# kouyt5/lightning-asr

Hardware: AMD Instinct MI355X
Metric: audio-seconds/sec training (asr13x1, bs=32, 10 s clips) (higher is better)
Workload: dtype bf16; 1 GPU; asr13x1 QuartzNet-CTC train step, bs=32/GPU, 10 s synthetic 16 kHz clips, labels.txt vocab (C=28), HIP mel+conv+CTC+NovoGrad, random-init weights; global_batch=32, n_class=28, parallelism=dp1, feature_prefetch=True, hip_graph=True, staged_backward=False

## Files before the change

### lightning_asr_amd/csrc/conv.hip

```cpp
#include "common.h"
#include "fused.h"

namespace lasr {

static thread_local const DwTapCtx* g_dw_tap_ctx = nullptr;
void dw_taps_set_ctx(const DwTapCtx* ctx) { g_dw_tap_ctx = ctx; }
bool dw_taps_enabled() {
  static const bool on = !(getenv("LASR_DW_TAPS") && atoi(getenv("LASR_DW_TAPS")) == 0);
  return on;
}
const uint32_t* dw_taps_for(const float* w, int flip, int64_t C) {
  (void)flip;
  const DwTapCtx* c = g_dw_tap_ctx;
  if (!c || C % 64 != 0) return nullptr;
  for (int i = 0; i < c->n; ++i)
    if (c->w[i] == w && c->C[i] == (int)C) return c->t[i];
  return nullptr;
}

static constexpr int kCB = 64;
static constexpr int kTT = 128;
static constexpr int kR = 8;
static constexpr int kMaxK = 128;

// ... 718 lines not shown
  __builtin_amdgcn_s_waitcnt(0);
#endif
  DW_STAMP(3);
}

template <int NKS, int NSET>
__global__ __launch_bounds__(512, 1) void dwconv_s1_mfma_kernel(const bf16_t* __restrict__ x, const float* __restrict__ w,
                                                                const bf16_t* __restrict__ addend, bf16_t* __restrict__ y,
                                                                int Tlen, int C, int k, int flip, const uint32_t* __restrict__ taps) {
  extern __shared__ __attribute__((aligned(16))) char smem_raw[];
  dwconv_s1_mfma_body<NKS, NSET>(x, w, addend, y, Tlen, C, k, flip, blockIdx.x, blockIdx.y, blockIdx.z, gridDim.z, smem_raw, taps);
}

template <int NKS, int NSET>
__global__ __launch_bounds__(512, 1) void dwconv_s1_mfma_bn_kernel(DwBnIn bn, const float* __restrict__ w, bf16_t* __restrict__ y, int Tlen,
                                                                   int C, int k, const uint32_t* __restrict__ taps) {
  extern __shared__ __attribute__((aligned(16))) char smem_raw[];
  dwconv_s1_mfma_body<NKS, NSET, true>(nullptr, w, nullptr, y, Tlen, C, k, 0, blockIdx.x, blockIdx.y, blockIdx.z, gridDim.z, smem_raw, taps, bn);
}

static constexpr int kSub = 32;

template <typename T>
__global__ __launch_bounds__(256) void dwconv_wgrad_s1_kernel(const T* __restrict__ x, const T* __restrict__ dy,
                                                              float* __restrict__ partials, int64_t Tlen, int64_t C, int k,
                                                              int ts) {
  extern __shared__ __attribute__((aligned(16))) char smem_raw[];
  const int pad = k / 2;
  const int ng = (k + 7) >> 3;
  const int kpad = ng * 8;
  const int WT = kSub * ts;
  const int in_rows = WT + kpad + 8;
  using P = S1<T>;
  constexpr int LD = P::kTileLd;
  T* s_x = reinterpret_cast<T*>(smem_raw);
  T* s_d = s_x + (size_t)in_rows * LD;
  const int b = blockIdx.z;
  const int64_t c0 = (int64_t)blockIdx.y * kCB;
  const int cl = threadIdx.x & 15, grp = threadIdx.x >> 4;
  const int jg = grp % ng, sp = grp / ng;
  const bool active = sp < ts;
  const T* xb = x + (int64_t)b * Tlen * C;
  const T* db = dy + (int64_t)b * Tlen * C;
  float4 acc[8];
#pragma unroll
  for (int j = 0; j < 8; ++j) acc[j] = make_float4(0.f, 0.f, 0.f, 0.f);
  const int64_t tbeg = (int64_t)blockIdx.x * kWChunk;
  const int64_t tend = tbeg + kWChunk < Tlen ? tbeg + kWChunk : Tlen;
  for (int64_t t0 = tbeg; t0 < tend; t0 += WT) {
    __syncthreads();
    const int64_t in0 = t0 - pad;
    {
      constexpr int kXP = (3 * kSub + kMaxK + 8 + P::kRowsPerPass - 1) / P::kRowsPerPass, kDP = (3 * kSub + P::kRowsPerPass - 1) / P::kRowsPerPass;
      const int lr = threadIdx.x / P::kLanesPerRow, lc = (threadIdx.x % P::kLanesPerRow) * P::kVec;
      const bool c_in = c0 + lc < C;
      uint4 vx[kXP], vd[kDP];
#pragma unroll
      for (int p = 0; p < kXP; ++p) {
        const int r = lr + p * P::kRowsPerPass;
        const int64_t ti = in0 + r;
        const uint4 ld = *reinterpret_cast<const uint4*>(xb + (int64_t)min(max(ti, (int64_t)0), Tlen - 1) * C + min(c0 + lc, C - P::kVec));
        const uint32_t mk = (r < in_rows && c_in && ti >= 0 && ti < Tlen) ? 0xffffffffu : 0u;
        vx[p] = make_uint4(ld.x & mk, ld.y & mk, ld.z & mk, ld.w & mk);
      }
#pragma unroll
      for (int p = 0; p < kDP; ++p) {
        const int r = lr + p * P::kRowsPerPass;
        const int64_t t = t0 + r;
        const uint4 ld = *reinterpret_cast<const uint4*>(db + (int64_t)min(t, Tlen - 1) * C + min(c0 + lc, C - P::kVec));
        const uint32_t mk = (r < WT && c_in && t < tend) ? 0xffffffffu : 0u;
        vd[p] = make_uint4(ld.x & mk, ld.y & mk, ld.z & mk, ld.w & mk);
      }
#pragma unroll
      for (int p = 0; p < kXP; ++p) {
        const int r = lr + p * P::kRowsPerPass;
        if (r < in_rows) *reinterpret_cast<uint4*>(s_x + (size_t)r * LD + lc) = vx[p];
      }
#pragma unroll
      for (int p = 0; p < kDP; ++p) {
        const int r = lr + p * P::kRowsPerPass;
        if (r < WT) *reinterpret_cast<uint4*>(s_d + (size_t)r * LD + lc) = vd[p];
      }
    }
    __syncthreads();
    if (active) {
      const T* xs = s_x + (size_t)(sp * kSub + jg * 8) * LD + cl * 4;
      const T* ds = s_d + (size_t)(sp * kSub) * LD + cl * 4;
      float4 win[8];
#pragma unroll
      for (int i = 0; i < 7; ++i) win[i] = lds_ld4<T>(xs + (size_t)i * LD);
      for (int tq = 0; tq < kSub; tq += 8) {
#pragma unroll
        for (int tt = 0; tt < 8; ++tt) {
          win[(tt + 7) & 7] = lds_ld4<T>(xs + (size_t)(tq + tt + 7) * LD);
          const float4 dv = lds_ld4<T>(ds + (size_t)(tq + tt) * LD);
#pragma unroll
          for (int jj = 0; jj < 8; ++jj) {
            const float4 xv = win[(tt + jj) & 7];
            acc[jj].x = fmaf(dv.x, xv.x, acc[jj].x);
            acc[jj].y = fmaf(dv.y, xv.y, acc[jj].y);
            acc[jj].z = fmaf(dv.z, xv.z, acc[jj].z);
            acc[jj].w = fmaf(dv.w, xv.w, acc[jj].w);
          }
        }
      }
    }
  }
  __syncthreads();
  float* s_red = reinterpret_cast<float*>(smem_raw);
  if (active) {
#pragma unroll
    for (int jj = 0; jj < 8; ++jj)
      *reinterpret_cast<float4*>(s_red + ((size_t)(sp * kpad + jg * 8 + jj)) * kCB + cl * 4) = acc[jj];
  }
  __syncthreads();
  float* out = partials + ((int64_t)b * gridDim.x + blockIdx.x) * C * k;
  for (int i = threadIdx.x; i < k * kCB; i += 256) {
    const int ch = i / k, j = i - ch * k;
    if (c0 + ch < C) {
      float s = 0.f;
      for (int q = 0; q < ts; ++q) s += s_red[((size_t)(q * kpad + j)) * kCB + ch];
      out[(c0 + ch) * k + j] = s;
    }
  }
}

namespace dwg {
static constexpr int TU = 288;
static constexpr int XF = TU + 16 * 7 + 8;
static constexpr int DF = TU + 16;
static constexpr int LDX = XF * 2;
static constexpr int LDD = DF * 2 + 16;
static constexpr int RSG = 256;
static constexpr int X_OFF = 0, D0_OFF = kCB * LDX;
static constexpr int ST_OFF = D0_OFF + kCB * LDD;
static constexpr int SMEM = ST_OFF + RSG * dwm::LDST;
static constexpr int XR = (XF + RSG - 1) / RSG, DR = (DF + RSG - 1) / RSG;
}

__device__ __forceinline__ void dwconv_wgrad_s1_mfma_body(const bf16_t* __restrict__ x, const bf16_t* __restrict__ dy,
                                                          float* __restrict__ partials, int Tlen, int C, int k, int bx, int by,
                                                          int bz, int gz, char* smem_raw) {
  using namespace dwg;
  char* ximg = smem_raw + X_OFF;
  char* d0 = smem_raw + D0_OFF;
  char* stage = smem_raw + ST_OFF;
  const int tid = threadIdx.x, lane = tid & 63, wid = tid >> 6;
  const int b = by, c0 = bx * kCB;
  const int pad = k / 2, P = (pad + 7) & ~7, sh = P - pad;
  const int n16 = lane & 15, g4 = lane >> 4;
  const bf16_t* xb = x + (size_t)b * Tlen * C;
  const bf16_t* db = dy + (size_t)b * Tlen * C;
  typedef __attribute__((address_space(3))) dw_s16x4 lds_s4;

  dw_f32x4 acc[8];
#pragma unroll
  for (int ch = 0; ch < 8; ++ch) acc[ch] = dw_f32x4{0.f, 0.f, 0.f, 0.f};
  for (int i = tid; i < kCB * 4; i += 512) *reinterpret_cast<uint32_t*>(d0 + (i >> 2) * LDD + DF * 2 + (i & 3) * 4) = 0u;

  const int n_tiles = (Tlen + 15 + TU) / TU;
  DW_STAMP(0);
  uint4 v[XR + DR][4];
  auto issue_loads = [&](int q) {
#pragma unroll
    for (int r = 0; r < XR + DR; ++r) {
#pragma unroll
      for (int h = 0; h < 4; ++h) {
        const int chk = tid + 512 * h;
        const bool isx = r < XR;
        const int fr = (isx ? r : r - XR) * RSG + (chk >> 3);
        const int t = isx ? TU * q + fr - P : TU * q - 16 + fr;
        const int cc = c0 + ((chk & 7) << 3);
        const bool ok = fr < (isx ? XF : DF) && t >= 0 && t < Tlen && cc < C;
        const bf16_t* src = isx ? xb : db;
        const uint4 ld = *reinterpret_cast<const uint4*>(src + (size_t)min(max(t, 0), Tlen - 1) * C + min(cc, C - 8));
        const uint32_t mk = ok ? 0xffffffffu : 0u;
        v[r][h] = make_uint4(ld.x & mk, ld.y & mk, ld.z & mk, ld.w & mk);
      }
    }
  };
  const int zq = bz, zn = gz;
  issue_loads(zq);
  for (int q = zq; q < n_tiles; q += zn) {
#pragma unroll
    for (int r = 0; r < XR + DR; ++r) {
      const bool isx = r < XR;
      const int rr = isx ? r : r - XR;
      __syncthreads();
#pragma unroll
      for (int h = 0; h < 4; ++h) {
        const int chk = tid + 512 * h;
        *reinterpret_cast<uint4*>(stage + (chk >> 3) * dwm::LDST + ((chk & 7) << 4)) = v[r][h];
      }
      __syncthreads();
      char* img = isx ? ximg : d0;
      const int ldi = isx ? LDX : LDD, nfr = isx ? XF : DF;
#pragma unroll
      for (int it = 0; it < 8; ++it) {
        const int blk = wid * 8 + it;
        const int fb = (blk >> 2) * 16 + g4 * 4, cg = blk & 3;
        const int qq = n16 >> 2, pp = n16 & 3;
        const dw_s16x4 d = __builtin_amdgcn_ds_read_tr16_b64_v4i16((lds_s4*)(stage + (fb + qq) * dwm::LDST + (cg * 16 + pp * 4) * 2));
        const int fr = rr * RSG + fb;
        if (fr < nfr) *reinterpret_cast<dw_s16x4*>(img + (cg * 16 + n16) * ldi + fr * 2) = d;
      }
    }
    __syncthreads();
    if (q == zq) DW_STAMP(1);
    if (q + zn < n_tiles) issue_loads(q + zn);
    if (q == zq) DW_STAMP(2);

#pragma unroll
    for (int ch = 0; ch < 8; ++ch) {
      const int cl = wid * 8 + ch;
      const int e0 = 8 * g4 - n16 + 16;
      const uint32_t shft = (e0 & 1) * 16;
      const uint32_t* arow = reinterpret_cast<const uint32_t*>(d0 + cl * LDD) + (e0 >> 1);
      const char* brow = ximg + cl * LDX + (16 * n16 + 8 * g4) * 2;
#pragma unroll
      for (int kb = 0; kb < TU / 32; kb += 3) {
        uint32_t wa[3][5];
        uint4 bb[3];
#pragma unroll
        for (int j = 0; j < 3; ++j) {
#pragma unroll
          for (int i = 0; i < 5; ++i) wa[j][i] = arow[16 * (kb + j) + i];
          bb[j] = *reinterpret_cast<const uint4*>(brow + 64 * (kb + j));
        }
#pragma unroll
        for (int j = 0; j < 3; ++j) {
          union { uint32_t u[4]; dw_bf16x8 v; } af, bf;
#pragma unroll
          for (int i = 0; i < 4; ++i) af.u[i] = __builtin_amdgcn_alignbit(wa[j][i + 1], wa[j][i], shft);
          bf.u[0] = bb[j].x; bf.u[1] = bb[j].y; bf.u[2] = bb[j].z; bf.u[3] = bb[j].w;
          acc[ch] = __builtin_amdgcn_mfma_f32_16x16x32_bf16(af.v, bf.v, acc[ch], 0, 0, 0);
        }
      }
    }
  }
  DW_STAMP(3);
  float* out = partials + ((size_t)b * zn + zq) * C * k;
#pragma unroll
  for (int ch = 0; ch < 8; ++ch) {
    const int c = c0 + wid * 8 + ch;
#pragma unroll
    for (int r = 0; r < 4; ++r) {
      const int j = 16 * n16 + 4 * g4 + r - sh;
      if (c < C && j >= 0 && j < k) out[(size_t)c * k + j] = acc[ch][r];
    }
  }
}

__global__ __launch_bounds__(512, 1) void dwconv_wgrad_s1_mfma_kernel(const bf16_t* __restrict__ x, const bf16_t* __restrict__ dy,
                                                                      float* __restrict__ partials, int Tlen, int C, int k) {
  extern __shared__ __attribute__((aligned(16))) char smem_raw[];
  dwconv_wgrad_s1_mfma_body(x, dy, partials, Tlen, C, k, blockIdx.x, blockIdx.y, blockIdx.z, gridDim.z, smem_raw);
}

struct DwBwd {
  const bf16_t* x; const bf16_t* dy; const float* w; const bf16_t* addend; bf16_t* dx; float* partials;
  int Tlen, C, k;
  int gx, B, gz_w, gz_d, n_w;
};
template <int NKS, int NSET>
__global__ __launch_bounds__(512, 1) void dwconv_bwd_s1_mfma_kernel(DwBwd a) {
  extern __shared__ __attribute__((aligned(16))) char smem_raw[];
  int id = blockIdx.x;
  if (id < a.n_w) {
    const int bx = id % a.gx, by = (id / a.gx) % a.B, bz = id / (a.gx * a.B);
    dwconv_wgrad_s1_mfma_body(a.x, a.dy, a.partials, a.Tlen, a.C, a.k, bx, by, bz, a.gz_w, smem_raw);
  } else {
    id -= a.n_w;
    const int bx = id % a.gx, by = (id / a.gx) % a.B, bz = id / (a.gx * a.B);
    dwconv_s1_mfma_body<NKS, NSET>(a.dy, a.w, a.addend, a.dx, a.Tlen, a.C, a.k, 1, bx, by, bz, a.gz_d, smem_raw, nullptr);
  }
}


__device__ __forceinline__ uint32_t dpp_row_shl(uint32_t v, int n) {
  switch (n) {
    case 0: return v;
    case 2: return (uint32_t)__builtin_amdgcn_update_dpp(0, (int)v, 0x102, 0xf, 0xf, true);
    case 4: return (uint32_t)__builtin_amdgcn_update_dpp(0, (int)v, 0x104, 0xf, 0xf, true);
    case 6: return (uint32_t)__builtin_amdgcn_update_dpp(0, (int)v, 0x106, 0xf, 0xf, true);
    case 8: return (uint32_t)__builtin_amdgcn_update_dpp(0, (int)v, 0x108, 0xf, 0xf, true);
    default: __builtin_unreachable();
  }
}

namespace dwu {
static constexpr int TT = 256;
static constexpr int FR = 384;
static constexpr int LDI = 784;
static constexpr int RS = 128;
template <int NKS, int NW>
struct Cfg {
  static constexpr int CB = 8 * NW, NT = 64 * NW;
  static constexpr int LDST = NW == 8 ? 160 : 96;
  static constexpr int WROW = 2 * (16 * NKS + 16);
  static constexpr int D_OFF = 0, X_OFF = CB * LDI, ST_OFF = 2 * CB * LDI, W_OFF = ST_OFF + RS * LDST;
  static constexpr int SMEM = W_OFF + CB * WROW * 4;
  static constexpr int LDO = CB * 2 + 16, LDOF = CB * 4 + 16;
  static_assert(TT * LDOF <= ST_OFF, "output image fits the two input images");
};
}

struct DwUni {
  const bf16_t* x; const bf16_t* dy; const float* w; const bf16_t* addend; bf16_t* dx; float* partials;
  int Tlen, C, k, gx, B, gz, total;
  const uint32_t* taps;
};

template <int NKS, int NW, bool NTL = false>
__global__ __launch_bounds__(64 * NW, NW == 8 ? 1 : 2) void dwconv_bwd_uni_kernel(DwUni a) {
  using K = dwu::Cfg<NKS, NW>;
  using namespace dwu;
  constexpr int CB = K::CB, NT = K::NT, LDST = K::LDST, WROW = K::WROW, HALF = WROW / 2, CG = CB / 16;
  extern __shared__ __attribute__((aligned(16))) char smem_raw[];
  int L;
  {
    const int id = blockIdx.x, xcd = id & 7, slot = id >> 3;
    L = NW == 8 ? id : (((slot >> 1) * 8 + xcd) * 2 + (slot & 1));
  }
  if (L >= a.total) return;
  const int bx = L % a.gx, by = (L / a.gx) % a.B, bz = L / (a.gx * a.B), gz = a.gz;
  char* dimg = smem_raw + K::D_OFF;
  char* ximg = smem_raw + K::X_OFF;
  char* stage = smem_raw + K::ST_OFF;
  uint32_t* wsm = reinterpret_cast<uint32_t*>(smem_raw + K::W_OFF);
  const int tid = threadIdx.x, lane = tid & 63, wid = tid >> 6;
  const int Tlen = a.Tlen, C = a.C, k = a.k;
  const int b = by, c0 = bx * CB;
  const int pad = k / 2, P = (pad + 7) & ~7, sh = P - pad;
  const int n16 = lane & 15, g4 = lane >> 4;
  const bf16_t* xb = a.x + (size_t)b * Tlen * C;
  const bf16_t* db = a.dy + (size_t)b * Tlen * C;
  const bf16_t* addend = a.addend;
  typedef __attribute__((address_space(3))) dw_s16x4 lds_s4;

  dw_f32x4 accw[8];
#pragma unroll
  for (int ch = 0; ch < 8; ++ch) accw[ch] = dw_f32x4{0.f, 0.f, 0.f, 0.f};

  const int n_tiles = (Tlen + TT - 1) / TT;
  constexpr int kRounds = FR / RS;
  uint4 vd[kRounds][2], vx[kRounds][2], ra[4];
  auto issue_loads = [&](int q) {
    const int tA = q * TT;
#pragma unroll
    for (int r = 0; r < kRounds; ++r) {
#pragma unroll
      for (int h = 0; h < 2; ++h) {
        const int ch = tid + NT * h;
        const int t = tA - P + r * RS + ch / NW;
        const int cc = c0 + (ch % NW) * 8;
        const size_t off = (size_t)min(max(t, 0), Tlen - 1) * C + min(cc, C - 8);
        vd[r][h] = *reinterpret_cast<const uint4*>(db + off);
        vx[r][h] = Vec<bf16_t>::raw_if_nt<NTL>(xb + off);
      }
    }
    if (addend) {
#pragma unroll
      for (int it = 0; it < 4; ++it) {
        const int ci = tid + NT * it;
        const int t = tA + ci / NW, cc = c0 + (ci % NW) * 8;
        ra[it] = Vec<bf16_t>::raw(addend + ((size_t)b * Tlen + min(t, Tlen - 1)) * C + min(cc, C - 8));
      }
    }
  };

  issue_loads(bz);
  if (a.taps) {
    constexpr int kV = CB * WROW / 4 / NT;
    static_assert(CB * WROW / 4 % NT == 0 && HALF % 4 == 0 && HALF <= kDwTapRow / 2, "tap table copy");
    uint4 tv[kV];
#pragma unroll
    for (int it = 0; it < kV; ++it) {
      const int i4 = tid + NT * it;
      const int ch = i4 / (WROW / 4), idx = (i4 - ch * (WROW / 4)) * 4;
      tv[it] = *reinterpret_cast<const uint4*>(a.taps + (size_t)(c0 + ch) * kDwTapRow + (idx < HALF ? idx : kDwTapRow / 2 + idx - HALF));
    }
#pragma unroll
    for (int it = 0; it < kV; ++it) reinterpret_cast<uint4*>(wsm)[tid + NT * it] = tv[it];
  } else {
    constexpr int kIt = CB * WROW / NT;
    float f0[kIt], f1[kIt];
#pragma unroll
    for (int it = 0; it < kIt; ++it) {
      const int i = tid + NT * it;
      const int ch = i / WROW, idx = i - ch * WROW;
      const int i0 = idx < HALF ? 2 * idx : 2 * (idx - HALF) + 1;
      const int j0 = i0 - 24, j1 = i0 - 23;
      const float* wc = a.w + (size_t)min(c0 + ch, C - 1) * k;
      const bool cok = c0 + ch < C;
      const int q0 = min(max(j0, 0), k - 1), q1 = min(max(j1, 0), k - 1);
      const float a0 = wc[k - 1 - q0], a1 = wc[k - 1 - q1];
      f0[it] = __uint_as_float(__float_as_uint(a0) & ((cok && j0 >= 0 && j0 < k) ? 0xffffffffu : 0u));
      f1[it] = __uint_as_float(__float_as_uint(a1) & ((cok && j1 >= 0 && j1 < k) ? 0xffffffffu : 0u));
    }
#pragma unroll
    for (int it = 0; it < kIt; ++it) wsm[tid + NT * it] = (uint32_t)f32_to_bf16(f0[it]) | ((uint32_t)f32_to_bf16(f1[it]) << 16);
  }

  DW_STAMP(0);
  for (int q = bz; q < n_tiles; q += gz) {
    const int tA = q * TT;
    const bool last = q == n_tiles - 1;
#pragma unroll
    for (int r2 = 0; r2 < 2 * kRounds; ++r2) {
      const bool isx = r2 >= kRounds;
      const int r = isx ? r2 - kRounds : r2;
      __syncthreads();
#pragma unroll
      for (int h = 0; h < 2; ++h) {
        const int ch = tid + NT * h;
        const int t = tA - P + r * RS + ch / NW;
        const uint32_t mk = (t >= 0 && t < Tlen && c0 + (ch % NW) * 8 < C) ? 0xffffffffu : 0u;
        const uint4 v = isx ? vx[r][h] : vd[r][h];
        *reinterpret_cast<uint4*>(stage + (ch / NW) * LDST + ((ch % NW) << 4)) = make_uint4(v.x & mk, v.y & mk, v.z & mk, v.w & mk);
      }
      __syncthreads();
      char* img = isx ? ximg : dimg;
#pragma unroll
      for (int it = 0; it < 4; ++it) {
        const int blk = wid * 4 + it;
        const int fb = (blk / CG) * 16 + g4 * 4, cg = blk % CG;
        const int qq = n16 >> 2, pp = n16 & 3;
        const dw_s16x4 d = __builtin_amdgcn_ds_read_tr16_b64_v4i16((lds_s4*)(stage + (fb + qq) * LDST + (cg * 16 + pp * 4) * 2));
        *reinterpret_cast<dw_s16x4*>(img + (cg * 16 + n16) * LDI + (r * RS + fb) * 2) = d;
      }
    }
    __syncthreads();
    const uint4 ra0 = ra[0], ra1 = ra[1], ra2 = ra[2], ra3 = ra[3];
    if (q == bz) DW_STAMP(1);
    if (q + gz < n_tiles) issue_loads(q + gz);
    if (q == bz) DW_STAMP(2);

    const int nku = last ? 9 : 8;
    (void)nku;
#ifndef LASR_DW_NO_BFRAG_DPP
    {
      constexpr int kDA = 4, NST = 64;
      const int e0 = P + 8 * g4 - n16;
      const uint32_t shft = (e0 & 1) * 16;
      const uint32_t* abase = reinterpret_cast<const uint32_t*>(dimg + wid * 8 * LDI) + (e0 >> 1);
      const char* bbase = ximg + wid * 8 * LDI + (16 * n16 + 8 * g4) * 2;
      auto ch_of = [](int i) { return 2 * (i >> 4) + (i & 1); };
      auto ks_of = [](int i) { return (i >> 1) & 7; };
      uint32_t wa[kDA][5];
      uint4 bq[2][2][2];
      auto issue_a = [&](int i, uint32_t (&dst)[5]) {
        const uint32_t* ar = abase + ch_of(i) * (LDI / 4) + 16 * ks_of(i);
#pragma unroll
        for (int d = 0; d < 5; ++d) dst[d] = ar[d];
      };
      auto issue_b = [&](int pair, uint4 (&dst)[2][2]) {
#pragma unroll
        for (int c2 = 0; c2 < 2; ++c2) {
          const char* br = bbase + (2 * pair + c2) * LDI;
          dst[c2][0] = *reinterpret_cast<const uint4*>(br);
          dst[c2][1] = *reinterpret_cast<const uint4*>(br + 64 * 4);
        }
      };
      issue_b(0, bq[0]);
#pragma unroll
      for (int i = 0; i < kDA; ++i) issue_a(i, wa[i]);
#pragma unroll
      for (int i = 0; i < NST; ++i) {
        const int ch = ch_of(i), ks = ks_of(i), pair = i >> 4;
        if ((i & 15) == 0 && pair + 1 < 4) issue_b(pair + 1, bq[(pair + 1) & 1]);
        union { uint32_t u[4]; dw_bf16x8 v; } af, bf;
#pragma unroll
        for (int d = 0; d < 4; ++d) af.u[d] = __builtin_amdgcn_alignbit(wa[i % kDA][d + 1], wa[i % kDA][d], shft);
        if (i + kDA < NST) issue_a(i + kDA, wa[i % kDA]);
        const uint4 base = bq[pair & 1][i & 1][ks >> 2];
        const int sft = 2 * (ks & 3);
        bf.u[0] = dpp_row_shl(base.x, sft); bf.u[1] = dpp_row_shl(base.y, sft);
        bf.u[2] = dpp_row_shl(base.z, sft); bf.u[3] = dpp_row_shl(base.w, sft);
        accw[ch] = __builtin_amdgcn_mfma_f32_16x16x32_bf16(af.v, bf.v, accw[ch], 0, 0, 0);
      }
      if (last) {
#pragma unroll
        for (int ch = 0; ch < 8; ++ch) {
          const uint32_t* ar = abase + ch * (LDI / 4) + 16 * 8;
          const uint4 bb = *reinterpret_cast<const uint4*>(bbase + ch * LDI + 64 * 8);
          uint32_t w9[5];
#pragma unroll
          for (int d = 0; d < 5; ++d) w9[d] = ar[d];
          union { uint32_t u[4]; dw_bf16x8 v; } af, bf;
#pragma unroll
          for (int d = 0; d < 4; ++d) af.u[d] = __builtin_amdgcn_alignbit(w9[d + 1], w9[d], shft);
          bf.u[0] = bb.x; bf.u[1] = bb.y; bf.u[2] = bb.z; bf.u[3] = bb.w;
          accw[ch] = __builtin_amdgcn_mfma_f32_16x16x32_bf16(af.v, bf.v, accw[ch], 0, 0, 0);
        }
      }
    }
#else
#pragma unroll
    for (int ch = 0; ch < 8; ++ch) {
      const int cl = wid * 8 + ch;
      const int e0 = P + 8 * g4 - n16;
      const uint32_t shft = (e0 & 1) * 16;
      const uint32_t* arow = reinterpret_cast<const uint32_t*>(dimg + cl * LDI) + (e0 >> 1);
      const char* brow = ximg + cl * LDI + (16 * n16 + 8 * g4) * 2;
#pragma unroll
      for (int kb = 0; kb < 9; kb += 3) {
        uint32_t wa[3][5];
        uint4 bb[3];
#pragma unroll
        for (int j = 0; j < 3; ++j) {
#pragma unroll
          for (int i = 0; i < 5; ++i) wa[j][i] = arow[16 * (kb + j) + i];
          bb[j] = *reinterpret_cast<const uint4*>(brow + 64 * (kb + j));
        }
#pragma unroll
        for (int j = 0; j < 3; ++j) {
          if (kb + j < nku) {
            union { uint32_t u[4]; dw_bf16x8 v; } af, bf;
#pragma unroll
            for (int i = 0; i < 4; ++i) af.u[i] = __builtin_amdgcn_alignbit(wa[j][i + 1], wa[j][i], shft);
            bf.u[0] = bb[j].x; bf.u[1] = bb[j].y; bf.u[2] = bb[j].z; bf.u[3] = bb[j].w;
            accw[ch] = __builtin_amdgcn_mfma_f32_16x16x32_bf16(af.v, bf.v, accw[ch], 0, 0, 0);
          }
        }
      }
    }
#endif
    if (q == bz) DW_STAMP(3);
    dw_f32x4 accd[8];
#pragma unroll
    for (int ch = 0; ch < 8; ++ch) accd[ch] = dw_f32x4{0.f, 0.f, 0.f, 0.f};
#pragma unroll
    for (int ch = 0; ch < 8; ++ch) {
      const int cl = wid * 8 + ch;
      const char* row = dimg + cl * LDI;
      const int s0 = 8 * g4 - n16 - sh + 24;
      const uint32_t* wrow = wsm + cl * WROW + ((s0 & 1) ? HALF + ((s0 - 1) >> 1) : (s0 >> 1));
      uint32_t wa[NKS][4];
      uint4 b0[NKS];
#pragma unroll
      for (int ks = 0; ks < NKS; ++ks) {
#pragma unroll
        for (int i = 0; i < 4; ++i) wa[ks][i] = wrow[16 * ks + i];
        b0[ks] = *reinterpret_cast<const uint4*>(row + (16 * n16 + 32 * ks + 8 * g4) * 2);
      }
#pragma unroll
      for (int ks = 0; ks < NKS; ++ks) {
        union { uint32_t u[4]; dw_bf16x8 v; } af, bf0;
#pragma unroll
        for (int i = 0; i < 4; ++i) af.u[i] = wa[ks][i];
        bf0.u[0] = b0[ks].x; bf0.u[1] = b0[ks].y; bf0.u[2] = b0[ks].z; bf0.u[3] = b0[ks].w;
        accd[ch] = __builtin_amdgcn_mfma_f32_16x16x32_bf16(af.v, bf0.v, accd[ch], 0, 0, 0);
      }
    }
    if (q == bz) DW_STAMP(4);
    __syncthreads();
    char* oimg = smem_raw;
#pragma unroll
    for (int r = 0; r < 4; ++r) {
      const int fl = n16 * 16 + g4 * 4 + r;
      const int prow = (fl & 15) * 16 + (fl >> 4);
      float o[8];
#pragma unroll
      for (int ch = 0; ch < 8; ++ch) o[ch] = accd[ch][r];
      if (!addend) {
        Vec<bf16_t>::store(reinterpret_cast<bf16_t*>(oimg + prow * K::LDO) + wid * 8, o);
      } else {
        *reinterpret_cast<float4*>(oimg + prow * K::LDOF + wid * 32) = make_float4(o[0], o[1], o[2], o[3]);
        *reinterpret_cast<float4*>(oimg + prow * K::LDOF + wid * 32 + 16) = make_float4(o[4], o[5], o[6], o[7]);
      }
    }
    __syncthreads();
    const uint4 rav[4] = {ra0, ra1, ra2, ra3};
#pragma unroll
    for (int it = 0; it < 4; ++it) {
      const int ci = tid + NT * it;
      const int fl = ci / NW, oc = ci % NW;
      const int t = tA + fl, cc = c0 + oc * 8;
      const bool ok = t < Tlen && cc < C;
      const size_t off = ((size_t)b * Tlen + min(t, Tlen - 1)) * C + min(cc, C - 8);
      const int prow = (fl & 15) * 16 + (fl >> 4);
      if (!addend) {
        if (ok) *reinterpret_cast<uint4*>(a.dx + off) = *reinterpret_cast<const uint4*>(oimg + prow * K::LDO + oc * 16);
      } else {
        const float4 lo = *reinterpret_cast<const float4*>(oimg + prow * K::LDOF + oc * 32);
        const float4 hi = *reinterpret_cast<const float4*>(oimg + prow * K::LDOF + oc * 32 + 16);
        float a8[8];
        Vec<bf16_t>::unpack(rav[it], a8);
        float o[8] = {lo.x + a8[0], lo.y + a8[1], lo.z + a8[2], lo.w + a8[3], hi.x + a8[4], hi.y + a8[5], hi.z + a8[6], hi.w + a8[7]};
        if (ok) Vec<bf16_t>::store(a.dx + off, o);
      }
    }
    if (q == bz) DW_STAMP(5);
  }
#ifdef LASR_DW_STAMPS
  __builtin_amdgcn_s_waitcnt(0);
#endif
  DW_STAMP(6);
  float* out = a.partials + ((size_t)b * gz + bz) * C * k;
#pragma unroll
  for (int ch = 0; ch < 8; ++ch) {
    const int c = c0 + wid * 8 + ch;
#pragma unroll
    for (int r = 0; r < 4; ++r) {
      const int j = 16 * n16 + 4 * g4 + r - sh;
      if (c < C && j >= 0 && j < k) out[(size_t)c * k + j] = accw[ch][r];
    }
  }
}

}

using namespace lasr;

static int64_t conv_out_len(int64_t Tin, int k, int stride) { return (Tin + 2 * (k / 2) - k) / stride + 1; }

extern "C" int lasr_dwconv_fwd(const void* x, const float* w, const void* addend, void* y, int dtype, int64_t B, int64_t Tin,
                               int64_t C, int k, int stride, int flip, void* stream) {
  LASR_CHECK_ARG(x && w && y, "lasr_dwconv_fwd: null pointer");
  LASR_CHECK_ARG(dtype == LASR_F32 || dtype == LASR_BF16, "lasr_dwconv_fwd: bad dtype");
  LASR_CHECK_SHAPE(k >= 1 && k <= kMaxK && (k & 1) && (stride == 1 || stride == 2) && C % 4 == 0 && B > 0 && B < 65536 && Tin > 0,
                   "lasr_dwconv_fwd: k=%d stride=%d C=%lld", k, stride, (long long)C);
  LASR_CHECK_SHAPE(!(flip && stride != 1), "lasr_dwconv_fwd: flip needs stride 1");
  LASR_CHECK_SHAPE(stride != 1 || (C % (int64_t)(16 / dtype_size(dtype)) == 0 && reinterpret_cast<uintptr_t>(x) % 16 == 0),
                   "lasr_dwconv_fwd: the stride-1 kernel loads 16-byte channel vectors (C=%lld)", (long long)C);
  const int64_t Tout = conv_out_len(Tin, k, stride);
  const int in_rows = (kTT - 1) * stride + k;
  const size_t shmem = ((size_t)in_rows + k) * kCB * sizeof(float);
  dim3 grid((unsigned)cdiv(Tout, kTT), (unsigned)cdiv(C, kCB), (unsigned)B);
  const int tok = prof_begin(LASR_PROF_DWCONV, as_stream(stream), 2.0 * (double)B * Tout * C * k,
                             (double)B * (Tin + Tout * (addend ? 2 : 1)) * C * dtype_size(dtype));
  if (stride == 1) {
    const int kpad = (k + 7) & ~7;
    const size_t esz1 = dtype_size(dtype);
    const size_t sh1 = (size_t)kpad * kCB * esz1 + (size_t)(kTT + kpad + 8) * (kCB + (esz1 == 2 ? 8 : 0)) * esz1;
    if (dtype == LASR_F32) {
      (void)hipFuncSetAttribute(reinterpret_cast<const void*>(dwconv_s1_kernel<float>), hipFuncAttributeMaxDynamicSharedMemorySize, 160 * 1024);
      hipLaunchKernelGGL(dwconv_s1_kernel<float>, grid, dim3(256), sh1, as_stream(stream), (const float*)x, w, (const float*)addend,
                         (float*)y, Tin, C, k, flip);
    } else {
      static const bool fma_form = getenv("LASR_DWCONV_FMA") != nullptr;
      static const bool dot2_form = getenv("LASR_DWCONV_DOT2") != nullptr;
      const int padk = k / 2, shk = ((padk + 7) & ~7) - padk;
      if (!fma_form && !dot2_form && C % 8 == 0 && 15 + k + shk <= dwm::KWMAX && Tin < (1 << 30)) {
        const int nks = (15 + k + shk + 31) / 32;
        static const bool no_half = getenv("LASR_DWCONV_NO_HALF") != nullptr;
        const bool half = !no_half && Tin > 256 && cdiv(C, kCB) * B * cdiv(Tin, (int64_t)512) < 200;
        const dim3 gridm((unsigned)cdiv(C, kCB), (unsigned)B, half ? (unsigned)std::min<int64_t>(cdiv(Tin, (int64_t)256), 8) : 1u);
        const uint32_t* taps = dw_taps_for(w, flip, C);
#define LASR_DWM2(N_, S_)                                                                                                    \
  do {                                                                                                                       \
    (void)hipFuncSetAttribute(reinterpret_cast<const void*>(dwconv_s1_mfma_kernel<N_, S_>), hipFuncAttributeMaxDynamicSharedMemorySize, 160 * 1024); \
    hipLaunchKernelGGL((dwconv_s1_mfma_kernel<N_, S_>), gridm, dim3(512), dwm::SMEM, as_stream(stream), (const bf16_t*)x, w,  \
                       (const bf16_t*)addend, (bf16_t*)y, (int)Tin, (int)C, k, flip, taps);                                  \
  } while (0)
#define LASR_DWM(N_) do { if (half) LASR_DWM2(N_, 1); else LASR_DWM2(N_, 2); } while (0)
        if (nks == 1) LASR_DWM(1); else if (nks == 2) LASR_DWM(2); else if (nks == 3) LASR_DWM(3); else LASR_DWM(4);
#undef LASR_DWM
#undef LASR_DWM2
      } else if (fma_form) {
        (void)hipFuncSetAttribute(reinterpret_cast<const void*>(dwconv_s1_kernel<bf16_t>), hipFuncAttributeMaxDynamicSharedMemorySize, 160 * 1024);
        hipLaunchKernelGGL(dwconv_s1_kernel<bf16_t>, grid, dim3(256), sh1, as_stream(stream), (const bf16_t*)x, w,
                           (const bf16_t*)addend, (bf16_t*)y, Tin, C, k, flip);
      } else {
        (void)hipFuncSetAttribute(reinterpret_cast<const void*>(dwconv_s1_bf16_kernel), hipFuncAttributeMaxDynamicSharedMemorySize, 160 * 1024);
        hipLaunchKernelGGL(dwconv_s1_bf16_kernel, grid, dim3(256), sh1, as_stream(stream), (const bf16_t*)x, w, (const bf16_t*)addend,
                           (bf16_t*)y, Tin, C, k, flip);
      }
    }
  } else {
    const bool small = (int64_t)grid.x * grid.y * grid.z < 200;
    const dim3 g2 = small ? dim3((unsigned)cdiv(Tout, 64), grid.y, grid.z) : grid;
#define LASR_DWF(T_, R_)                                                                                                          \
  do {                                                                                                                            \
    (void)hipFuncSetAttribute(reinterpret_cast<const void*>(dwconv_fwd_kernel<T_, R_>), hipFuncAttributeMaxDynamicSharedMemorySize, 160 * 1024); \
    hipLaunchKernelGGL((dwconv_fwd_kernel<T_, R_>), g2, dim3(256), shmem, as_stream(stream), (const T_*)x, w, (const T_*)addend, (T_*)y, Tin,  \
                       Tout, C, k, stride, flip);                                                                                 \
  } while (0)
    if (dtype == LASR_F32) { if (small) LASR_DWF(float, 4); else LASR_DWF(float, 8); }
    else { if (small) LASR_DWF(bf16_t, 4); else LASR_DWF(bf16_t, 8); }
#undef LASR_DWF
  }
  prof_end(tok, as_stream(stream));
  LASR_LAUNCH_CHECK("dwconv_fwd_kernel");
  return 0;
}

int lasr::dwconv_fwd_bn(const void* y, const float* coef, const void* y2, const float* coef2, int act, const float* w, void* out, void* u,
                        int64_t B, int64_t T, int64_t C, int k, void* stream) {
  LASR_CHECK_ARG(y && coef && w && out && u && (!y2 || coef2), "dwconv_fwd_bn: null pointer");
  static const bool off = getenv("LASR_DWCONV_FMA") || getenv("LASR_DWCONV_DOT2");
  const int padk = k / 2, shk = ((padk + 7) & ~7) - padk;
  auto al16 = [](const void* p) { return reinterpret_cast<uintptr_t>(p) % 16 == 0; };
  if (off || k < 1 || k > kMaxK || !(k & 1) || C % 8 != 0 || C < 8 || 15 + k + shk > dwm::KWMAX || T <= 0 || T >= (1 << 30) || B <= 0 ||
      B >= 65536 || !al16(y) || !al16(y2) || !al16(out) || !al16(u) || !al16(coef) || !al16(coef2))
    return 1;
  const int nks = (15 + k + shk + 31) / 32;
  static const bool no_half = getenv("LASR_DWCONV_NO_HALF") != nullptr;
  const bool half = !no_half && T > 256 && cdiv(C, kCB) * B * cdiv(T, (int64_t)512) < 200;
  static const bool full_too = getenv("LASR_BN_DW_FUSE") && atoi(getenv("LASR_BN_DW_FUSE")) == 2;
  if (!half && !full_too) return 1;
  const dim3 gridm((unsigned)cdiv(C, kCB), (unsigned)B, half ? (unsigned)std::min<int64_t>(cdiv(T, (int64_t)256), 8) : 1u);
  DwBnIn bn;
  bn.y = (const bf16_t*)y; bn.y2 = (const bf16_t*)y2; bn.coef = coef; bn.coef2 = coef2; bn.out = (bf16_t*)out; bn.act = act;
  const int tok = prof_begin(LASR_PROF_DWCONV, as_stream(stream), 2.0 * (double)B * T * C * k, (double)B * T * C * (y2 ? 4 : 3) * 2);
  const uint32_t* taps = dw_taps_for(w, 0, C);
#define LASR_DWMB2(N_, S_)                                                                                                  \
  do {                                                                                                                      \
    (void)hipFuncSetAttribute(reinterpret_cast<const void*>(dwconv_s1_mfma_bn_kernel<N_, S_>), hipFuncAttributeMaxDynamicSharedMemorySize, 160 * 1024); \
    hipLaunchKernelGGL((dwconv_s1_mfma_bn_kernel<N_, S_>), gridm, dim3(512), dwm::SMEM, as_stream(stream), bn, w, (bf16_t*)u, (int)T, (int)C, k, taps); \
  } while (0)
#define LASR_DWMB(N_) do { if (half) LASR_DWMB2(N_, 1); else LASR_DWMB2(N_, 2); } while (0)
  if (nks == 1) LASR_DWMB(1); else if (nks == 2) LASR_DWMB(2); else if (nks == 3) LASR_DWMB(3); else LASR_DWMB(4);
#undef LASR_DWMB
#undef LASR_DWMB2
  prof_end(tok, as_stream(stream));
  LASR_LAUNCH_CHECK("dwconv_s1_mfma_bn_kernel");
  return 0;
}

extern "C" size_t lasr_dwconv_wgrad_workspace_bytes(int64_t B, int64_t Tout, int64_t C, int k) {
  return (size_t)B * cdiv(Tout, kWChunkG) * C * k * sizeof(float);
}

static int dwconv_wgrad_impl(const void* x, const void* dy, float* dw, int dtype, int64_t B, int64_t Tin, int64_t C, int k,
                            int stride, void* workspace, size_t workspace_bytes, void* stream, int* n_partials_out);

extern "C" int lasr_dwconv_wgrad(const void* x, const void* dy, float* dw, int dtype, int64_t B, int64_t Tin, int64_t C, int k,
                                 int stride, void* workspace, size_t workspace_bytes, void* stream) {
  LASR_CHECK_ARG(dw, "lasr_dwconv_wgrad: null pointer");
  return dwconv_wgrad_impl(x, dy, dw, dtype, B, Tin, C, k, stride, workspace, workspace_bytes, stream, nullptr);
}

extern "C" int lasr_dwconv_wgrad_partials(const void* x, const void* dy, int dtype, int64_t B, int64_t Tin, int64_t C, int k,
                                          int stride, void* workspace, size_t workspace_bytes, int* n_partials, void* stream) {
  LASR_CHECK_ARG(n_partials, "lasr_dwconv_wgrad_partials: null pointer");
  return dwconv_wgrad_impl(x, dy, nullptr, dtype, B, Tin, C, k, stride, workspace, workspace_bytes, stream, n_partials);
}

static int dwconv_wgrad_impl(const void* x, const void* dy, float* dw, int dtype, int64_t B, int64_t Tin, int64_t C, int k,
                             int stride, void* workspace, size_t workspace_bytes, void* stream, int* n_partials_out) {
  LASR_CHECK_ARG(x && dy && workspace, "lasr_dwconv_wgrad: null pointer");
  LASR_CHECK_ARG(dtype == LASR_F32 || dtype == LASR_BF16, "lasr_dwconv_wgrad: bad dtype");
  LASR_CHECK_SHAPE(k >= 1 && k <= kMaxK && (k & 1) && (stride == 1 || stride == 2) && C % 4 == 0 && B > 0 && B < 65536 && Tin > 0,
                   "lasr_dwconv_wgrad: k=%d stride=%d C=%lld", k, stride, (long long)C);
  const int64_t Tout = conv_out_len(Tin, k, stride);
  if (workspace_bytes < lasr_dwconv_wgrad_workspace_bytes(B, Tout, C, k)) return fail(LASR_E_WORKSPACE, "lasr_dwconv_wgrad: workspace");
  {
    static const bool valu_form = getenv("LASR_DWWGRAD_VALU") != nullptr;
    const int padk = k / 2, shk = ((padk + 7) & ~7) - padk;
    if (!valu_form && stride == 1 && dtype == LASR_BF16 && C % 8 == 0 && k + shk <= 16 * 7 && Tin < (1 << 30)) {
      float* parts = reinterpret_cast<float*>(workspace);
      const int n_tiles = (int)((Tin + 15 + dwg::TU) / dwg::TU);
      static const int zmax = getenv("LASR_DWWGRAD_ZSPLIT") ? atoi(getenv("LASR_DWWGRAD_ZSPLIT")) : 2;
      int zsplit = 1;
      while (zsplit < zmax && zsplit * 2 <= n_tiles && cdiv(C, kCB) * B * zsplit < 200) zsplit *= 2;
      (void)hipFuncSetAttribute(reinterpret_cast<const void*>(dwconv_wgrad_s1_mfma_kernel), hipFuncAttributeMaxDynamicSharedMemorySize, 160 * 1024);
      hipLaunchKernelGGL(dwconv_wgrad_s1_mfma_kernel, dim3((unsigned)cdiv(C, kCB), (unsigned)B, (unsigned)zsplit), dim3(512), dwg::SMEM,
                         as_stream(stream), (const bf16_t*)x, (const bf16_t*)dy, parts, (int)Tin, (int)C, k);
      LASR_LAUNCH_CHECK("dwconv_wgrad_s1_mfma_kernel");
      if (n_partials_out) { *n_partials_out = (int)B * zsplit; return 0; }
      return launch_reduce_partials(parts, (int)B * zsplit, C * k, dw, C * k, nullptr, as_stream(stream));
    }
  }
  const int n_chunks = (int)cdiv(Tout, stride == 1 ? kWChunk : kWChunkG);
  const int in_rows = (kWT - 1) * stride + k;
  const size_t shmem = ((size_t)in_rows + kWT) * kCB * sizeof(float);
  dim3 grid((unsigned)n_chunks, (unsigned)cdiv(C, kCB), (unsigned)B);
  float* partials = reinterpret_cast<float*>(workspace);
  if (stride == 1) {
    const int ng = (k + 7) >> 3;
    int ts = 16 / ng;
    if (ts > 3) ts = 3;
    const int WT = kSub * ts, kpad = ng * 8;
    size_t sh1 = (size_t)(WT + kpad + 8 + WT) * (kCB + (dtype_size(dtype) == 2 ? 8 : 0)) * dtype_size(dtype);
    const size_t red = (size_t)ts * kpad * kCB * sizeof(float);
    if (red > sh1) sh1 = red;
    if (dtype == LASR_F32) {
      (void)hipFuncSetAttribute(reinterpret_cast<const void*>(dwconv_wgrad_s1_kernel<float>), hipFuncAttributeMaxDynamicSharedMemorySize, 160 * 1024);
      hipLaunchKernelGGL(dwconv_wgrad_s1_kernel<float>, grid, dim3(256), sh1, as_stream(stream), (const float*)x, (const float*)dy,
                         partials, Tin, C, k, ts);
    } else {
      (void)hipFuncSetAttribute(reinterpret_cast<const void*>(dwconv_wgrad_s1_kernel<bf16_t>), hipFuncAttributeMaxDynamicSharedMemorySize, 160 * 1024);
      hipLaunchKernelGGL(dwconv_wgrad_s1_kernel<bf16_t>, grid, dim3(256), sh1, as_stream(stream), (const bf16_t*)x, (const bf16_t*)dy,
                         partials, Tin, C, k, ts);
    }
  } else if (dtype == LASR_F32) {
    (void)hipFuncSetAttribute(reinterpret_cast<const void*>(dwconv_wgrad_kernel<float>), hipFuncAttributeMaxDynamicSharedMemorySize, 160 * 1024);
    hipLaunchKernelGGL(dwconv_wgrad_kernel<float>, grid, dim3(256), shmem, as_stream(stream), (const float*)x, (const float*)dy,
                       partials, Tin, Tout, C, k, stride);
  } else {
    (void)hipFuncSetAttribute(reinterpret_cast<const void*>(dwconv_wgrad_kernel<bf16_t>), hipFuncAttributeMaxDynamicSharedMemorySize, 160 * 1024);
    hipLaunchKernelGGL(dwconv_wgrad_kernel<bf16_t>, grid, dim3(256), shmem, as_stream(stream), (const bf16_t*)x,
                       (const bf16_t*)dy, partials, Tin, Tout, C, k, stride);
  }
  LASR_LAUNCH_CHECK("dwconv_wgrad_kernel");
  const int64_t n = C * k;
  if (n_partials_out) { *n_partials_out = (int)(B * n_chunks); return 0; }
  return launch_reduce_partials(partials, (int)(B * n_chunks), n, dw, n, nullptr, as_stream(stream));
}

#ifdef LASR_DW_STAMPS
extern "C" int lasr_debug_set_dw_stamps(void* buf) {
  unsigned long long* p = reinterpret_cast<unsigned long long*>(buf);
  return (int)hipMemcpyToSymbol(HIP_SYMBOL(lasr::g_dw_stamps), &p, sizeof(p));
}
#endif

extern "C" int lasr_dwconv_bwd_fused(const void* x, const void* dy, const float* w, const void* addend, void* dx, int dtype,
                                     int64_t B, int64_t T, int64_t C, int k, void* workspace, size_t workspace_bytes,
                                     int* n_partials, void* stream) {
  LASR_CHECK_ARG(x && dy && w && dx && workspace && n_partials, "lasr_dwconv_bwd_fused: null pointer");
  LASR_CHECK_ARG(dtype == LASR_F32 || dtype == LASR_BF16, "lasr_dwconv_bwd_fused: bad dtype");
  LASR_CHECK_SHAPE(k >= 1 && k <= kMaxK && (k & 1) && C % 4 == 0 && B > 0 && B < 65536 && T > 0, "lasr_dwconv_bwd_fused: k=%d C=%lld", k,
                   (long long)C);
  const int padk = k / 2, shk = ((padk + 7) & ~7) - padk;
  static const bool no_fused = getenv("LASR_DW_NO_FUSED_BWD") != nullptr;
  static const bool valu = getenv("LASR_DWWGRAD_VALU") || getenv("LASR_DWCONV_FMA") || getenv("LASR_DWCONV_DOT2");
  const bool ok = !no_fused && !valu && dtype == LASR_BF16 && C % 8 == 0 && 15 + k + shk <= dwm::KWMAX && k + shk <= 16 * 7 &&
                  T < (1 << 30) && reinterpret_cast<uintptr_t>(x) % 16 == 0 && reinterpret_cast<uintptr_t>(dy) % 16 == 0 &&
                  workspace_bytes >= lasr_dwconv_wgrad_workspace_bytes(B, T, C, k);
  if (!ok) {
    LASR_TRY(lasr_dwconv_wgrad_partials(x, dy, dtype, B, T, C, k, 1, workspace, workspace_bytes, n_partials, stream));
    return lasr_dwconv_fwd(dy, w, addend, dx, dtype, B, T, C, k, 1, 1, stream);
  }
  const int nks = (15 + k + shk + 31) / 32;
  {
    static const int uni = getenv("LASR_DW_UNI") ? atoi(getenv("LASR_DW_UNI")) : 32;
    const bool u32 = uni == 32 && nks <= 3;
    if (uni == 64 || uni == 32) {
      DwUni u;
      u.x = (const bf16_t*)x; u.dy = (const bf16_t*)dy; u.w = w; u.addend = (const bf16_t*)addend; u.dx = (bf16_t*)dx;
      u.partials = reinterpret_cast<float*>(workspace);
      u.Tlen = (int)T; u.C = (int)C; u.k = k; u.B = (int)B;
      {
        const uint32_t* tp = dw_taps_for(w, 1, C);
        u.taps = tp ? tp + (size_t)C * kDwTapRow : nullptr;
      }
      const int cb = u32 ? 32 : 64;
      u.gx = (int)cdiv(C, cb);
      const int n_tiles = (int)cdiv(T, (int64_t)dwu::TT);
      const int want = u32 ? 400 : 200;
      int gz = 1;
      while (gz * 2 <= n_tiles && (int64_t)u.gx * B * gz < want) gz *= 2;
      u.gz = gz;
      u.total = (int)(u.gx * B * gz);
      const int tok = prof_begin(LASR_PROF_DWCONV, as_stream(stream), 4.0 * (double)B * T * C * k, (double)B * T * C * (addend ? 4 : 3) * 2);
      const bool ntl = (nt_loads_mask() & 4) != 0;
#define LASR_DWU(N_, W_) do { if (ntl) LASR_DWU2(N_, W_, true); else LASR_DWU2(N_, W_, false); } while (0)
#define LASR_DWU2(N_, W_, NT_)                                                                                                    \
  do {                                                                                                                            \
    using Kc = dwu::Cfg<N_, W_>;                                                                                                  \
    (void)hipFuncSetAttribute(reinterpret_cast<const void*>(dwconv_bwd_uni_kernel<N_, W_, NT_>), hipFuncAttributeMaxDynamicSharedMemorySize, 160 * 1024); \
    const unsigned grid = (unsigned)((u.total + 15) / 16 * 16);                                                                     \
    hipLaunchKernelGGL((dwconv_bwd_uni_kernel<N_, W_, NT_>), dim3(grid), dim3(64 * W_), Kc::SMEM, as_stream(stream), u);             \
  } while (0)
      if (u32) { if (nks == 1) LASR_DWU(1, 4); else if (nks == 2) LASR_DWU(2, 4); else LASR_DWU(3, 4); }
      else { if (nks == 1) LASR_DWU(1, 8); else if (nks == 2) LASR_DWU(2, 8); else if (nks == 3) LASR_DWU(3, 8); else LASR_DWU(4, 8); }
#undef LASR_DWU
#undef LASR_DWU2
      prof_end(tok, as_stream(stream));
      LASR_LAUNCH_CHECK("dwconv_bwd_uni_kernel");
      *n_partials = (int)B * gz;
      return 0;
    }
  }
  DwBwd a;
  a.x = (const bf16_t*)x; a.dy = (const bf16_t*)dy; a.w = w; a.addend = (const bf16_t*)addend; a.dx = (bf16_t*)dx;
  a.partials = reinterpret_cast<float*>(workspace);
  a.Tlen = (int)T; a.C = (int)C; a.k = k; a.gx = (int)cdiv(C, kCB); a.B = (int)B;
  const int n_tiles = (int)((T + 15 + dwg::TU) / dwg::TU);
  static const int zmax = getenv("LASR_DWWGRAD_ZSPLIT") ? atoi(getenv("LASR_DWWGRAD_ZSPLIT")) : 2;
  int zsplit = 1;
  while (zsplit < zmax && zsplit * 2 <= n_tiles && cdiv(C, kCB) * B * zsplit < 200) zsplit *= 2;
  a.gz_w = zsplit;
  a.n_w = a.gx * a.B * a.gz_w;
  static const bool no_half = getenv("LASR_DWCONV_NO_HALF") != nullptr;
  const bool half = !no_half && T > 256 && cdiv(C, kCB) * B * cdiv(T, (int64_t)512) < 200;
  a.gz_d = half ? (int)std::min<int64_t>(cdiv(T, (int64_t)256), 8) : 1;
  const unsigned total = (unsigned)(a.n_w + a.gx * a.B * a.gz_d);
  constexpr int kSmem = dwm::SMEM > dwg::SMEM ? dwm::SMEM : dwg::SMEM;
  const int tok = prof_begin(LASR_PROF_DWCONV, as_stream(stream), 4.0 * (double)B * T * C * k, (double)B * T * C * (addend ? 5 : 4) * 2);
#define LASR_DWB2(N_, S_)                                                                                                      \
  do {                                                                                                                         \
    (void)hipFuncSetAttribute(reinterpret_cast<const void*>(dwconv_bwd_s1_mfma_kernel<N_, S_>), hipFuncAttributeMaxDynamicSharedMemorySize, 160 * 1024); \
    hipLaunchKernelGGL((dwconv_bwd_s1_mfma_kernel<N_, S_>), dim3(total), dim3(512), kSmem, as_stream(stream), a);                \
  } while (0)
#define LASR_DWB(N_) do { if (half) LASR_DWB2(N_, 1); else LASR_DWB2(N_, 2); } while (0)
  if (nks == 1) LASR_DWB(1); else if (nks == 2) LASR_DWB(2); else if (nks == 3) LASR_DWB(3); else LASR_DWB(4);
#undef LASR_DWB
#undef LASR_DWB2
  prof_end(tok, as_stream(stream));
  LASR_LAUNCH_CHECK("dwconv_bwd_s1_mfma_kernel");
  *n_partials = (int)B * zsplit;
  return 0;
}
```

Before: 159,800 audio-seconds/sec.

## Stage depthwise-conv backward inputs via LDS-DMA ring in 32-channel kernel

For the 32-channel form of the unified depthwise-conv backward kernel, global loads of dy and x now go straight into LDS through global_load_lds_dwordx4 instead of through registers. They use a three-slot 4 KiB ring in the staging region, with vmcnt waits and prefetch two rounds ahead. The addend load is moved after staging, and boundary masking moves to the transpose-read step. This aims to cut register pressure and the VGPR round trip of the staging path, at the cost of inline asm touching m0 and delicate vmcnt accounting. It is on by default and can be disabled with LASR_DW_BWD_DMA=0.

```diff
diff --git a/lightning_asr_amd/csrc/conv.hip b/lightning_asr_amd/csrc/conv.hip
--- a/lightning_asr_amd/csrc/conv.hip
+++ b/lightning_asr_amd/csrc/conv.hip
@@ -1044,7 +1044,21 @@
   static constexpr int SMEM = W_OFF + CB * WROW * 4;
   static constexpr int LDO = CB * 2 + 16, LDOF = CB * 4 + 16;
   static_assert(TT * LDOF <= ST_OFF, "output image fits the two input images");
+  static constexpr int SF = 64, SLOT = SF * 64, NSL = RS * LDST / SLOT, NRD = 2 * FR / SF;
+  static_assert(NW != 4 || (NSL == 3 && NRD == 12), "DMA ring: three 4 KiB slots in the 12 KiB staging region");
 };
+template <bool NT>
+__device__ __forceinline__ void glds16(const void* gsrc, uint32_t lds) {
+  uint32_t keep;
+  if constexpr (NT)
+    asm volatile("s_mov_b32 %0, m0\n\ts_mov_b32 m0, %2\n\ts_nop 0\n\tglobal_load_lds_dwordx4 %1, off nt\n\ts_mov_b32 m0, %0"
+                 : "=&s"(keep) : "v"(gsrc), "s"(lds) : "memory");
+  else
+    asm volatile("s_mov_b32 %0, m0\n\ts_mov_b32 m0, %2\n\ts_nop 0\n\tglobal_load_lds_dwordx4 %1, off\n\ts_mov_b32 m0, %0"
+                 : "=&s"(keep) : "v"(gsrc), "s"(lds) : "memory");
+}
+template <int N>
+__device__ __forceinline__ void vm_wait() { asm volatile("s_waitcnt vmcnt(%0)" : : "n"(N) : "memory"); }
 }
 
 struct DwUni {
@@ -1053,10 +1067,11 @@
   const uint32_t* taps;
 };
 
-template <int NKS, int NW, bool NTL = false>
+template <int NKS, int NW, bool NTL = false, bool DMA = false>
 __global__ __launch_bounds__(64 * NW, NW == 8 ? 1 : 2) void dwconv_bwd_uni_kernel(DwUni a) {
   using K = dwu::Cfg<NKS, NW>;
   using namespace dwu;
+  static_assert(!DMA || NW == 4, "LDS-DMA staging: 32-channel form");
   constexpr int CB = K::CB, NT = K::NT, LDST = K::LDST, WROW = K::WROW, HALF = WROW / 2, CG = CB / 16;
   extern __shared__ __attribute__((aligned(16))) char smem_raw[];
   int L;
@@ -1087,10 +1102,31 @@
   const int n_tiles = (Tlen + TT - 1) / TT;
   constexpr int kRounds = FR / RS;
   uint4 vd[kRounds][2], vx[kRounds][2], ra[4];
+  const uint32_t st_lds = (uint32_t)(size_t)(__attribute__((address_space(3))) char*)stage + __builtin_amdgcn_readfirstlane(wid) * 1024;
+  auto dma_round = [&](int q, int j) {
+    const int row = 16 * wid + (lane >> 2), pc = lane & 3;
+    const int oct = (pc ^ ((lane >> 3) & 2));
+    const int t = q * TT - P + (j % 6) * K::SF + row;
+    const size_t off = (size_t)min(max(t, 0), Tlen - 1) * C + min(c0 + 8 * oct, C - 8);
+    const uint32_t dst = st_lds + (j % K::NSL) * K::SLOT;
+    if (j < 6) glds16<false>(db + off, dst);
+    else glds16<NTL>(xb + off, dst);
+  };
+  auto issue_addend = [&](int q) {
+    if (addend) {
+      const int tA = q * TT;
+#pragma unroll
+      for (int it = 0; it < 4; ++it) {
+        const int ci = tid + NT * it;
+        const int t = tA + ci / NW, cc = c0 + (ci % NW) * 8;
+        ra[it] = Vec<bf16_t>::raw(addend + ((size_t)b * Tlen + min(t, Tlen - 1)) * C + min(cc, C - 8));
+      }
+    }
+  };
   auto issue_loads = [&](int q) {
     const int tA = q * TT;
 #pragma unroll
-    for (int r = 0; r < kRounds; ++r) {
+    for (int r = 0; r < (DMA ? 0 : kRounds); ++r) {
 #pragma unroll
       for (int h = 0; h < 2; ++h) {
         const int ch = tid + NT * h;
@@ -1101,13 +1137,11 @@
         vx[r][h] = Vec<bf16_t>::raw_if_nt<NTL>(xb + off);
       }
     }
-    if (addend) {
-#pragma unroll
-      for (int it = 0; it < 4; ++it) {
-        const int ci = tid + NT * it;
-        const int t = tA + ci / NW, cc = c0 + (ci % NW) * 8;
-        ra[it] = Vec<bf16_t>::raw(addend + ((size_t)b * Tlen + min(t, Tlen - 1)) * C + min(cc, C - 8));
-      }
+    if constexpr (DMA) {
+#pragma unroll
+      for (int j = 0; j < K::NSL; ++j) dma_round(q, j);
+    } else {
+      issue_addend(q);
     }
   };
 
@@ -1148,6 +1182,36 @@
   for (int q = bz; q < n_tiles; q += gz) {
     const int tA = q * TT;
     const bool last = q == n_tiles - 1;
+    if constexpr (DMA) {
+      const bool sb = q != bz && c0 + CB <= C;
+#pragma unroll
+      for (int j = 0; j < K::NRD; ++j) {
+        if (j == 0) { if (sb) vm_wait<6>(); else vm_wait<2>(); }
+        else if (j <= 2) { if (sb) vm_wait<5>(); else vm_wait<1>(); }
+        else if (j < K::NRD - 1) vm_wait<1>();
+        else vm_wait<0>();
+        __syncthreads();
+        if (j >= 1 && j + 2 < K::NRD) dma_round(q, j + 2);
+        const char* slot = stage + (j % K::NSL) * K::SLOT;
+        char* img = j < 6 ? dimg : ximg;
+        const int f0 = (j % 6) * K::SF;
+#pragma unroll
+        for (int it = 0; it < 2; ++it) {
+          const int blk = wid * 2 + it;
+          const int fb = (blk >> 1) * 16 + g4 * 4, cg = blk & 1;
+          const int qq = n16 >> 2, pp = n16 & 3;
+          union { dw_s16x4 v; uint32_t u[2]; } d;
+          d.v = __builtin_amdgcn_ds_read_tr16_b64_v4i16((lds_s4*)(slot + (fb + qq) * 64 + ((cg ^ (g4 & 1)) * 32) + pp * 8));
+          const int tf = tA - P + f0 + fb;
+          const bool cok = c0 + cg * 16 + n16 < C;
+          const uint32_t mk0 = (cok && (unsigned)tf < (unsigned)Tlen ? 0xffffu : 0u) | (cok && (unsigned)(tf + 1) < (unsigned)Tlen ? 0xffff0000u : 0u);
+          const uint32_t mk1 = (cok && (unsigned)(tf + 2) < (unsigned)Tlen ? 0xffffu : 0u) | (cok && (unsigned)(tf + 3) < (unsigned)Tlen ? 0xffff0000u : 0u);
+          d.u[0] &= mk0;
+          d.u[1] &= mk1;
+          *reinterpret_cast<dw_s16x4*>(img + (cg * 16 + n16) * LDI + (f0 + fb) * 2) = d.v;
+        }
+      }
+    } else {
 #pragma unroll
     for (int r2 = 0; r2 < 2 * kRounds; ++r2) {
       const bool isx = r2 >= kRounds;
@@ -1172,7 +1236,9 @@
         *reinterpret_cast<dw_s16x4*>(img + (cg * 16 + n16) * LDI + (r * RS + fb) * 2) = d;
       }
     }
+    }
     __syncthreads();
+    if constexpr (DMA) issue_addend(q);
     const uint4 ra0 = ra[0], ra1 = ra[1], ra2 = ra[2], ra3 = ra[3];
     if (q == bz) DW_STAMP(1);
     if (q + gz < n_tiles) issue_loads(q + gz);
@@ -1589,16 +1655,21 @@
       u.total = (int)(u.gx * B * gz);
       const int tok = prof_begin(LASR_PROF_DWCONV, as_stream(stream), 4.0 * (double)B * T * C * k, (double)B * T * C * (addend ? 4 : 3) * 2);
       const bool ntl = (nt_loads_mask() & 4) != 0;
-#define LASR_DWU(N_, W_) do { if (ntl) LASR_DWU2(N_, W_, true); else LASR_DWU2(N_, W_, false); } while (0)
-#define LASR_DWU2(N_, W_, NT_)                                                                                                    \
+      static const bool dma = !(getenv("LASR_DW_BWD_DMA") && atoi(getenv("LASR_DW_BWD_DMA")) == 0);
+#define LASR_DWU(N_, W_, DMA_) do { if (ntl) LASR_DWU2(N_, W_, true, DMA_); else LASR_DWU2(N_, W_, false, DMA_); } while (0)
+#define LASR_DWU2(N_, W_, NT_, DMA_)                                                                                              \
   do {                                                                                                                            \
     using Kc = dwu::Cfg<N_, W_>;                                                                                                  \
-    (void)hipFuncSetAttribute(reinterpret_cast<const void*>(dwconv_bwd_uni_kernel<N_, W_, NT_>), hipFuncAttributeMaxDynamicSharedMemorySize, 160 * 1024); \
+    (void)hipFuncSetAttribute(reinterpret_cast<const void*>(dwconv_bwd_uni_kernel<N_, W_, NT_, DMA_>), hipFuncAttributeMaxDynamicSharedMemorySize, 160 * 1024); \
     const unsigned grid = (unsigned)((u.total + 15) / 16 * 16);                                                                     \
-    hipLaunchKernelGGL((dwconv_bwd_uni_kernel<N_, W_, NT_>), dim3(grid), dim3(64 * W_), Kc::SMEM, as_stream(stream), u);             \
+    hipLaunchKernelGGL((dwconv_bwd_uni_kernel<N_, W_, NT_, DMA_>), dim3(grid), dim3(64 * W_), Kc::SMEM, as_stream(stream), u);       \
   } while (0)
-      if (u32) { if (nks == 1) LASR_DWU(1, 4); else if (nks == 2) LASR_DWU(2, 4); else LASR_DWU(3, 4); }
-      else { if (nks == 1) LASR_DWU(1, 8); else if (nks == 2) LASR_DWU(2, 8); else if (nks == 3) LASR_DWU(3, 8); else LASR_DWU(4, 8); }
+      if (u32 && dma) { if (nks == 1) LASR_DWU(1, 4, true); else if (nks == 2) LASR_DWU(2, 4, true); else LASR_DWU(3, 4, true); }
+      else if (u32) { if (nks == 1) LASR_DWU(1, 4, false); else if (nks == 2) LASR_DWU(2, 4, false); else LASR_DWU(3, 4, false); }
+      else {
+        if (nks == 1) LASR_DWU(1, 8, false); else if (nks == 2) LASR_DWU(2, 8, false); else if (nks == 3) LASR_DWU(3, 8, false);
+        else LASR_DWU(4, 8, false);
+      }
 #undef LASR_DWU
 #undef LASR_DWU2
       prof_end(tok, as_stream(stream));
```

After: 161,800 audio-seconds/sec, median of 6. 1.01x the previous value.
